# polimi-ispl/deep_prior_interpolation

Hardware: AMD Instinct MI355X
Metric: Adam iters/sec on 3D MultiRes-UNet (whole job over n_gpus; per_gpu beside it); recon SNR(dB) vs ref under config.snr_vs_reference (higher is better)
Workload: dtype f32

## Files before the change

deep_prior_interpolation_amd/csrc/conv_mfma.hip:

```cpp
#include "conv_kernels.h"

namespace {

typedef float f32x4 __attribute__((ext_vector_type(4)));

struct MArgs {
  const float* __restrict__ x;
  const float* __restrict__ chain;
  const float* __restrict__ w;
  const float* __restrict__ bias;
  float* __restrict__ y;
  double* __restrict__ partials;
  int Cin, Cout;
  int D, H, W;
  int ntd, nth, ntw;
  long w_out_stride, w_in_stride;
  int accumulate;
  int split_cps;
  const float* __restrict__ x2;
  const float* __restrict__ w2;
  int C2;
  long w2_co_stride, w2_c_stride;
  int xb, yb;
  int ny;
};

template <int KD, int NR, int NH, int S = 1>
struct Geo {
  static constexpr bool SLICES = (KD == 3 && NR >= 4);
  static constexpr int SD = KD == 3 ? S : 1;
  static constexpr int TZ = SLICES ? 4 : 1;
  static constexpr int TY = SLICES ? NR : 4 * NR;
  static constexpr int TW = 16 * NH;
  static constexpr int ID = (TZ - 1) * SD + KD;
  static constexpr int IH = (TY - 1) * S + 3;
  static constexpr int IW = (TW - 1) * S + 3;
  static constexpr int RS = (IW + 3) & ~3;
  static constexpr int DS0 = IH * RS;
  static constexpr int DS = (S == 1 && (RS % 32) == 4) ? DS0 + ((12 - (DS0 % 32)) + 32) % 32 : DS0;
  static constexpr int CS0 = ID * DS;
  static constexpr int CSM = S == 1 ? 16 : 1;
  static constexpr int CS = CS0 + ((CSM - (CS0 % 32)) + 32) % 32;
  static constexpr int TILE = ID * IH * IW;
  static constexpr int E = (TILE + 255) / 256;
  static constexpr int NROW = (NR - 1) * S + 3;
  static constexpr int NSTEP = KD * NROW;
  static constexpr int NB = 3 * NH;
};

__device__ __forceinline__ int xcd_tile(int bid, int ntiles) {
  const int q = ntiles >> 3, r = ntiles & 7, xcd = bid & 7, i = bid >> 3;
  return (xcd < r ? xcd * (q + 1) : r * (q + 1) + (xcd - r) * q) + i;
}

template <class G>
__device__ __forceinline__ void tile_slots(int tid, int id0, int ih0, int iw0, int D, int H, int W, int (&goff)[G::E], int (&loff)[G::E]) {
#pragma unroll
  for (int e = 0; e < G::E; ++e) {
    const int idx = tid + e * 256;
    const int col = idx % G::IW, row = idx / G::IW;
    const int hy = row % G::IH, dz = row / G::IH;
    const int gd = id0 + dz, gh = ih0 + hy, gw = iw0 + col;
    const bool ok = idx < G::TILE && gd >= 0 && gd < D && gh >= 0 && gh < H && gw >= 0 && gw < W;
    goff[e] = ok ? (gd * H + gh) * W + gw : -1;
    loff[e] = idx < G::TILE ? dz * G::DS + hy * G::RS + col : -1;
  }
}

template <class G>
__device__ __forceinline__ void stage_load(float (&sr)[4][G::E], const float* __restrict__ x, int Cin, size_t V, int c0,
                                           const int (&goff)[G::E], bool xb = false) {
  if (xb) {
#pragma unroll
    for (int c = 0; c < 4; ++c) {
      const int ci = min(c0 + c, Cin - 1);
      const __amdgpu_buffer_rsrc_t r = dpi_buffer_t(dpi_at(x, (size_t)ci * V, true), V, true);
#pragma unroll
      for (int e = 0; e < G::E; ++e) sr[c][e] = dpi_buffer_load_bf16_raw(r, goff[e]);
    }
    return;
  }
#pragma unroll
  for (int c = 0; c < 4; ++c) {
    const int ci = min(c0 + c, Cin - 1);
    const __amdgpu_buffer_rsrc_t r = dpi_buffer(x + (size_t)ci * V, V * sizeof(float));
#pragma unroll
    for (int e = 0; e < G::E; ++e) sr[c][e] = dpi_buffer_load(r, goff[e] * 4);
  }
}

template <class G>
__device__ __forceinline__ void stage_store(float* lds, const float (&sr_in)[4][G::E], const float* __restrict__ chain, int Cin, int c0,
                                            const int (&goff)[G::E], const int (&loff)[G::E], bool xb = false) {
  float sr[4][G::E];
#pragma unroll
  for (int c = 0; c < 4; ++c)
#pragma unroll
    for (int e = 0; e < G::E; ++e) sr[c][e] = sr_in[c][e];
  if (xb) {
#pragma unroll
    for (int c = 0; c < 4; ++c)
#pragma unroll
      for (int e = 0; e < G::E; ++e) sr[c][e] = dpi_widen_raw(sr[c][e]);
  }
  if (chain == nullptr) {
#pragma unroll
    for (int c = 0; c < 4; ++c)
// ... 11 lines not shown
      const float v = goff[e] >= 0 ? apply_chain(t, sr[c][e]) : sr[c][e];
      if ((e + 1) * 256 <= G::TILE || loff[e] >= 0) lds[c * G::CS + loff[e]] = v;
    }
  }
}

template <int KD, int NR, int NH>
struct GeoV2 {
  static constexpr int TY = 4 * NR, TW = 16 * NH;
  static constexpr int ID = KD == 3 ? 3 : 1, IH = (TY - 1) * 2 + 3;
  static constexpr int NQ = TW / 2 + 1;
  static constexpr int PW = 2 * NQ;
  static constexpr int RS = 2 * PW;
  static constexpr int DS = IH * RS;
  static constexpr int CS0 = ID * DS;
  static constexpr int CS = CS0 + ((16 - (CS0 % 32)) + 32) % 32;
  static constexpr int NV4 = ID * IH * NQ;
  static constexpr int E = (NV4 + 255) / 256;
};
template <class GV>
__device__ __forceinline__ void tile_slots_v(int tid, int id0, int ih0, int iw0, int D, int H, int W, int (&goff)[GV::E], int (&loff)[GV::E]) {
#pragma unroll
  for (int e = 0; e < GV::E; ++e) {
    const int idx = tid + e * 256;
    const int q = idx % GV::NQ, row = idx / GV::NQ;
    const int hy = row % GV::IH, dz = row / GV::IH;
    const int gd = id0 + dz, gh = ih0 + hy, gw = iw0 + 4 * q;
    const bool ok = idx < GV::NV4 && gd >= 0 && gd < D && gh >= 0 && gh < H && gw >= 0 && gw + 4 <= W;
    goff[e] = ok ? (gd * H + gh) * W + gw : -4;
    loff[e] = idx < GV::NV4 ? dz * GV::DS + hy * GV::RS + 2 * q : -1;
  }
}
template <class GV>
__device__ __forceinline__ void stage_load_v(f32x4 (&sv)[4][GV::E], const float* __restrict__ x, int Cin, size_t V, int c0, const int (&goff)[GV::E]) {
#pragma unroll
  for (int c = 0; c < 4; ++c) {
    const int ci = min(c0 + c, Cin - 1);
    const __amdgpu_buffer_rsrc_t r = dpi_buffer(x + (size_t)ci * V, V * sizeof(float));
#pragma unroll
    for (int e = 0; e < GV::E; ++e) sv[c][e] = __builtin_bit_cast(f32x4, __builtin_amdgcn_raw_buffer_load_b128(r, goff[e] * 4, 0, 0));
  }
}
template <class GV>
__device__ __forceinline__ void stage_store_v(float* lds, const f32x4 (&sv)[4][GV::E], const float* __restrict__ chain, int Cin, int c0,
                                              const int (&goff)[GV::E], const int (&loff)[GV::E]) {
  typedef float f32x2 __attribute__((ext_vector_type(2)));
  if (chain == nullptr) {
#pragma unroll
    for (int c = 0; c < 4; ++c)
#pragma unroll
      for (int e = 0; e < GV::E; ++e)
        if ((e + 1) * 256 <= GV::NV4 || loff[e] >= 0) {
          float* const p = lds + c * GV::CS + loff[e];
          *reinterpret_cast<f32x2*>(p) = (f32x2){sv[c][e][0], sv[c][e][2]};
          *reinterpret_cast<f32x2*>(p + GV::PW) = (f32x2){sv[c][e][1], sv[c][e][3]};
        }
    return;
  }
#pragma unroll
  for (int c = 0; c < 4; ++c) {
    const Chain t = load_chain(chain, min(c0 + c, Cin - 1));
#pragma unroll
    for (int e = 0; e < GV::E; ++e) {
      const float m = goff[e] >= 0 ? 1.f : 0.f;
      if ((e + 1) * 256 <= GV::NV4 || loff[e] >= 0) {
        float* const p = lds + c * GV::CS + loff[e];
        *reinterpret_cast<f32x2*>(p) = (f32x2){m * apply_chain(t, sv[c][e][0]), m * apply_chain(t, sv[c][e][2])};
        *reinterpret_cast<f32x2*>(p + GV::PW) = (f32x2){m * apply_chain(t, sv[c][e][1]), m * apply_chain(t, sv[c][e][3])};
      }
    }
  }
}

#ifdef DPI_TRACE
__device__ long long g_blk[8192][4];
__device__ long long g_trace[4][64];
#define TR(i) do { if (trc >= 0 && tid == 0) g_trace[trc][i] = clock64(); } while (0)
#define TRC(i) do { if (trc >= 0 && tid == 0 && (i) < 38) g_trace[trc][i] = clock64(); } while (0)
#else
#define TR(i)
#define TRC(i)
#endif
template <int KD, int NR, int NH, bool FLIP, int S = 1, int WPE = 2, bool PERSIST = false, bool TAILPACK = false, bool IOB = false, bool YLOOP = false,
          bool S2V = false>
__global__ __launch_bounds__(256, WPE) void conv_mfma_kernel(MArgs a) {
  static_assert(!YLOOP || (!PERSIST && !TAILPACK), "the channel-tile loop is built for the one-tile-per-workgroup variants without a packed tail");
  static_assert(!S2V || (S == 2 && !FLIP && !PERSIST && !TAILPACK && !IOB && NR < 4), "vectorised stride-2 staging: forward, fp32 tensors, row-split tiles");
  using GV = GeoV2<KD, NR < 4 ? NR : 2, NH>;
  if constexpr (!IOB) { a.xb = 0; a.yb = 0; }
  using G = Geo<KD, NR, NH, S>;
  constexpr int TAPS = KD * 9;
  constexpr int PD = (KD - 1) / 2;
  constexpr int NT = NR * NH;
  __shared__ __attribute__((aligned(16))) float lds[4 * (S2V ? GV::CS : G::CS)];
  __shared__ double red[4][16][2];

  const int tid = threadIdx.x, lane = tid & 63, wid = tid >> 6;
  const int lk = lane >> 4, lj = lane & 15;
  const int ntiles = a.ntd * a.nth * a.ntw;
  int vt0 = blockIdx.x, ytile = blockIdx.y;
  if constexpr (!PERSIST) {
    if (a.ny > 0) {
      const int q8 = ntiles >> 3, r8 = ntiles & 7, xcd = blockIdx.x & 7, j = blockIdx.x >> 3;
      const int i = YLOOP ? j : j / a.ny;
      ytile = YLOOP ? 0 : j - i * a.ny;
      if (i >= q8 + (xcd < r8 ? 1 : 0)) return;
      vt0 = i * 8 + xcd;
    }
  }
  int n0 = ytile * 16;
  const size_t V = (size_t)a.D * a.H * a.W;
  const int Do = (a.D + 2 * PD - KD) / G::SD + 1, Ho = (a.H - 1) / S + 1, Wo = (a.W - 1) / S + 1;
  const size_t Vo = (size_t)Do * Ho * Wo;
#ifdef DPI_TRACE
  const int trc = blockIdx.y != 0 ? -1 : blockIdx.x == 0 ? 0 : blockIdx.x == 1 ? 1 : blockIdx.x == 30 ? 2 : blockIdx.x == 50 ? 3 : -1;
  TR(0);
  if (tid == 0 && blockIdx.y == 0 && blockIdx.x < 8192) {
    g_blk[blockIdx.x][0] = wall_clock64();
    g_blk[blockIdx.x][2] = __builtin_amdgcn_s_getreg(63492);
    g_blk[blockIdx.x][3] = __builtin_amdgcn_s_getreg(63508);
  }
#endif
  auto tile_origin = [&](int vt, int& tile_id, int& od0, int& oh0, int& ow0) {
    tile_id = xcd_tile(vt, ntiles);
    int bt = tile_id;
    const int tw_i = bt % a.ntw; bt /= a.ntw;
    const int th_i = bt % a.nth; bt /= a.nth;
    od0 = bt * G::TZ; oh0 = th_i * G::TY; ow0 = tw_i * G::TW;
  };

  const int wz = G::SLICES ? wid : 0, wh = G::SLICES ? 0 : wid * NR;
  const int lbase = S2V ? lk * GV::CS + wh * 2 * GV::RS + lj : lk * G::CS + wz * G::SD * G::DS + wh * S * G::RS + lj * S;

  int co_w = n0 + lj;
  auto w_ptr = [&](int c0, bool& ok) {
    const int ci = c0 + lk;
    ok = co_w < a.Cout && ci < a.Cin;
    return a.w + (ok ? co_w : 0) * a.w_out_stride + (ok ? ci : 0) * a.w_in_stride;
  };
  auto load_w_raw = [&](float (&wn)[9], int c0, int kd) {
    bool ok;
    const float* __restrict__ wp = w_ptr(c0, ok);
#pragma unroll
    for (int t = 0; t < 9; ++t) wn[t] = wp[FLIP ? (TAPS - 1 - (kd * 9 + t)) : kd * 9 + t];
  };
  auto commit_w = [&](float (&wr)[TAPS], const float (&wn)[9], int c0, int kd) {
    const bool ok = co_w < a.Cout && c0 + lk < a.Cin;
#pragma unroll
    for (int t = 0; t < 9; ++t) wr[kd * 9 + t] = ok ? wn[t] : 0.f;
  };

  const int c_lo = a.split_cps ? (int)blockIdx.z * a.split_cps : 0;
  float* __restrict__ const ybase = a.y + (size_t)blockIdx.z * a.Cout * Vo;
  constexpr int EE = S2V ? GV::E : G::E;
  int goff[EE], loff[EE];
  float wr[TAPS], wn[9], sr[S2V ? 1 : 4][S2V ? 1 : G::E];
  f32x4 sv[S2V ? 4 : 1][S2V ? GV::E : 1];
  auto slots = [&](int od, int oh, int ow) {
    if constexpr (S2V) tile_slots_v<GV>(tid, od * G::SD - PD, oh * 2 - 1, ow * 2 - 4, a.D, a.H, a.W, goff, loff);
    else tile_slots<G>(tid, od * G::SD - PD, oh * S - 1, ow * S - 1, a.D, a.H, a.W, goff, loff);
  };
  auto sload = [&](int c0) {
    if constexpr (S2V) stage_load_v<GV>(sv, a.x, a.Cin, V, c0, goff);
    else stage_load<G>(sr, a.x, a.Cin, V, c0, goff, a.xb);
  };
  auto sstore = [&](int c0) {
    if constexpr (S2V) stage_store_v<GV>(lds, sv, a.chain, a.Cin, c0, goff, loff);
    else stage_store<G>(lds, sr, a.chain, a.Cin, c0, goff, loff, a.xb);
  };
  int vt = vt0, tile_id, od0, oh0, ow0;
  tile_origin(vt, tile_id, od0, oh0, ow0);
  slots(od0, oh0, ow0);
  sload(c_lo);
  {
    bool ok;
    const float* __restrict__ wp = w_ptr(c_lo, ok);
#pragma unroll
    for (int t = 0; t < TAPS; ++t) wr[t] = wp[FLIP ? (TAPS - 1 - t) : t];
#pragma unroll
    for (int t = 0; t < TAPS; ++t) wr[t] = ok ? wr[t] : 0.f;
  }

  constexpr int NTG = (TAPS + 3) / 4;
  const bool tail = TAILPACK && S == 1 && (a.Cin & 3) == 1 && (a.Cin > 4 || a.Cin == 1);
  const int cin_main = a.split_cps ? min(c_lo + a.split_cps, a.Cin) : (tail ? a.Cin - 1 : a.Cin);
  int ttoff[TAILPACK ? NTG : 1];
  float wt[TAILPACK ? NTG : 1];
  if constexpr (TAILPACK) {
#pragma unroll
    for (int g = 0; g < NTG; ++g) {
      const int t = 4 * g + lk;
      const int kd = t / 9, kh = (t / 3) % 3, kw = t % 3;
      ttoff[g] = t < TAPS ? kd * G::DS + kh * G::RS + kw : 0;
      wt[g] = 0.f;
    }
  }
  auto load_tail_w = [&]() {
    if constexpr (TAILPACK) {
      const bool ok = co_w < a.Cout;
      const float* __restrict__ wp = a.w + (ok ? co_w : 0) * a.w_out_stride + (a.Cin - 1) * a.w_in_stride;
#pragma unroll
      for (int g = 0; g < NTG; ++g) {
        const int t = 4 * g + lk < TAPS ? 4 * g + lk : TAPS - 1;
        wt[g] = wp[FLIP ? (TAPS - 1 - t) : t];
      }
    }
  };
  auto commit_tail_w = [&]() {
    if constexpr (TAILPACK) {
#pragma unroll
      for (int g = 0; g < NTG; ++g) wt[g] = (co_w < a.Cout && 4 * g + lk < TAPS) ? wt[g] : 0.f;
    }
  };

  for (;;) {
    const int vt_next = vt + (int)gridDim.x;
    const bool has_next = PERSIST && vt_next < ntiles;
    int tile_n = 0, od_n = 0, oh_n = 0, ow_n = 0;
    if (has_next) tile_origin(vt_next, tile_n, od_n, oh_n, ow_n);

    const int nyt = YLOOP ? a.ny : 1;
    for (int yt = 0; yt < nyt; ++yt) {
    if constexpr (YLOOP) {
      if (yt > 0) {
        n0 = yt * 16; co_w = n0 + lj;
        const bool ok = co_w < a.Cout && c_lo + lk < a.Cin;
#pragma unroll
        for (int t = 0; t < TAPS; ++t) wr[t] = ok ? wr[t] : 0.f;
      }
    }
    f32x4 acc[NT];
#pragma unroll
    for (int t = 0; t < NT; ++t) acc[t] = (f32x4){0.f, 0.f, 0.f, 0.f};
    if (a.accumulate) {
#pragma unroll
      for (int r = 0; r < 4; ++r) {
        const int co = n0 + 4 * lk + r;
#pragma unroll
        for (int t = 0; t < NT; ++t) {
          const int od = od0 + wz, oh = oh0 + wh + t / NH, ow = ow0 + (t % NH) * 16 + lj;
          if (co < a.Cout && od < Do && oh < Ho && ow < Wo) acc[t][r] = dpi_ld(ybase, (size_t)co * Vo + ((size_t)od * Ho + oh) * Wo + ow, a.yb);
        }
      }
    }

    TR(1);
    for (int c0 = c_lo; c0 < cin_main; c0 += 4) {
      if (!YLOOP || yt == 0) {
      __syncthreads();
      TRC(2 + (c0 / 4) * 4);
      sstore(c0);
      TRC(3 + (c0 / 4) * 4);
      __syncthreads();
      TRC(4 + (c0 / 4) * 4);
      }
      const bool more = c0 + 4 < cin_main;
      const bool tail_next = tail && !more;
      if (more || tail_next) sload(c0 + 4);
      else if (has_next) {
        slots(od_n, oh_n, ow_n);
        sload(c_lo);
      }
      float bc[G::NB], bn[G::NB];
      auto load_b = [&](float (&b)[G::NB], int step) {
        const int kd = step / G::NROW, ir = step % G::NROW;
#pragma unroll
        for (int h = 0; h < NH; ++h)
#pragma unroll
          for (int kw = 0; kw < 3; ++kw) {
            if constexpr (S2V)
              b[h * 3 + kw] = lds[lbase + kd * GV::DS + ir * GV::RS + h * 16 + (kw == 1 ? 2 : GV::PW + (kw == 0 ? 1 : 2))];
            else b[h * 3 + kw] = lds[lbase + kd * G::DS + ir * G::RS + h * 16 * S + kw];
          }
      };
      load_b(bc, 0);
      const int cn = more ? c0 + 4 : c_lo;
      if (tail_next) load_tail_w();
#pragma unroll
      for (int step = 0; step < G::NSTEP; ++step) {
        const int kd = step / G::NROW, ir = step % G::NROW;
        if (step + 1 < G::NSTEP) load_b(bn, step + 1);
        if constexpr (!YLOOP) { if (ir == 0) load_w_raw(wn, cn, kd); }
        if (WPE <= 2) __builtin_amdgcn_sched_barrier(0);
#pragma unroll
        for (int kw = 0; kw < 3; ++kw)
#pragma unroll
          for (int kh = 0; kh < 3; ++kh) {
            const int hr = (ir - kh) / S;
            if (ir - kh >= 0 && (ir - kh) % S == 0 && hr < NR) {
#pragma unroll
              for (int h = 0; h < NH; ++h)
                acc[hr * NH + h] = __builtin_amdgcn_mfma_f32_16x16x4f32(wr[(kd * 3 + kh) * 3 + kw], bc[h * 3 + kw], acc[hr * NH + h], 0, 0, 0);
            }
          }
        if (WPE <= 2) __builtin_amdgcn_sched_barrier(0);
#pragma unroll
        for (int i = 0; i < G::NB; ++i) bc[i] = bn[i];
        if constexpr (!YLOOP) { if (ir == G::NROW - 1) commit_w(wr, wn, cn, kd); }
      }
      if (tail_next) commit_tail_w();
      TRC(5 + (c0 / 4) * 4);
    }
    if constexpr (TAILPACK) {
      if (tail && cin_main == 0) { load_tail_w(); commit_tail_w(); }
      if (tail) {
        __syncthreads();
        sstore(cin_main);
        __syncthreads();
        if (has_next) {
          slots(od_n, oh_n, ow_n);
          sload(0);
        }
#pragma unroll
        for (int hr = 0; hr < NR; ++hr) {
          float tb[NH][NTG];
#pragma unroll
          for (int h = 0; h < NH; ++h)
#pragma unroll
            for (int g = 0; g < NTG; ++g) tb[h][g] = lds[lbase + ttoff[g] + hr * G::RS + h * 16];
#pragma unroll
          for (int g = 0; g < NTG; ++g)
#pragma unroll
            for (int h = 0; h < NH; ++h)
              acc[hr * NH + h] = __builtin_amdgcn_mfma_f32_16x16x4f32(wt[g], tb[h][g], acc[hr * NH + h], 0, 0, 0);
        }
      }
    }
    if constexpr (YLOOP) {
      if (yt + 1 < nyt) {
        const int con = (yt + 1) * 16 + lj, ci = c_lo + lk;
        const bool okn = con < a.Cout && ci < a.Cin;
        const float* __restrict__ wp = a.w + (okn ? con : 0) * a.w_out_stride + (okn ? ci : 0) * a.w_in_stride;
#pragma unroll
        for (int t = 0; t < TAPS; ++t) wr[t] = wp[FLIP ? (TAPS - 1 - t) : t];
      }
    }
    if constexpr (FLIP && !PERSIST) if (a.x2 != nullptr) {
      const __amdgpu_buffer_rsrc_t r2 = dpi_buffer_t(a.x2, (size_t)a.C2 * Vo, a.xb);
      int voff[NT];
#pragma unroll
      for (int t = 0; t < NT; ++t) {
        const int od = od0 + wz, oh = oh0 + wh + t / NH, ow = ow0 + (t % NH) * 16 + lj;
        voff[t] = (od < Do && oh < Ho && ow < Wo) ? (od * Ho + oh) * Wo + ow : -1;
      }
      const int nk2 = (a.C2 + 3) >> 2;
      auto load2 = [&](float (&b)[NT], float& wv, int kc) {
        const int c = kc * 4 + lk;
        const bool ok = c < a.C2 && co_w < a.Cout;
        const float wraw = a.w2[(ok ? co_w : 0) * a.w2_co_stride + (ok ? c : 0) * a.w2_c_stride];
        wv = ok ? wraw : 0.f;
        const int cbase = c * (int)Vo;
#pragma unroll
        for (int t = 0; t < NT; ++t)
          b[t] = a.xb ? dpi_buffer_load_bf16(r2, voff[t] >= 0 ? cbase + voff[t] : -1) : dpi_buffer_load(r2, voff[t] >= 0 ? (cbase + voff[t]) * 4 : -4);
      };
      float b0[NT], b1[NT], w0v, w1v;
      load2(b0, w0v, 0);
      for (int kc = 0; kc < nk2; kc += 2) {
        if (kc + 1 < nk2) load2(b1, w1v, kc + 1);
#pragma unroll
        for (int t = 0; t < NT; ++t) acc[t] = __builtin_amdgcn_mfma_f32_16x16x4f32(w0v, b0[t], acc[t], 0, 0, 0);
        if (kc + 1 < nk2) {
          if (kc + 2 < nk2) load2(b0, w0v, kc + 2);
#pragma unroll
          for (int t = 0; t < NT; ++t) acc[t] = __builtin_amdgcn_mfma_f32_16x16x4f32(w1v, b1[t], acc[t], 0, 0, 0);
        }
      }
    }
    TR(40);

    const bool interior = od0 + G::TZ <= Do && oh0 + G::TY <= Ho && ow0 + G::TW <= Wo && n0 + 16 <= a.Cout;
    const int vbase = ((od0 + wz) * Ho + oh0 + wh) * Wo + ow0 + lj;
#pragma unroll
    for (int r = 0; r < 4; ++r) {
      const int co = n0 + 4 * lk + r;
      const bool cok = co < a.Cout;
      const float bv = (a.bias && cok) ? a.bias[co] : 0.f;
      float* __restrict__ yc = dpi_at(ybase, (size_t)(cok ? co : 0) * Vo + vbase, a.yb);
      double s = 0.0, q = 0.0;
      if (a.yb) {
        const bool pairs = !(Wo & 1) && !(Vo & 1) && !((uintptr_t)ybase & 3);
#pragma unroll
        for (int t = 0; t < NT; ++t) {
          const int od = od0 + wz, oh = oh0 + wh + t / NH, ow = ow0 + (t % NH) * 16 + lj;
          const bool ok = interior || (cok && od < Do && oh < Ho && ow < Wo);
          const float v = dpi_round_bf16(acc[t][r] + bv);
          dpi_st_bf16_row(yc, (t / NH) * Wo + (t % NH) * 16, v, ok, pairs, lj);
          if (ok) { s += v; q += (double)v * v; }
        }
      } else if (interior) {
#pragma unroll
        for (int t = 0; t < NT; ++t) {
          const float v = acc[t][r] + bv;
          yc[(t / NH) * Wo + (t % NH) * 16] = v;
          if (a.partials) { s += v; q += (double)v * v; }
        }
      } else {
#pragma unroll
        for (int t = 0; t < NT; ++t) {
          const int od = od0 + wz, oh = oh0 + wh + t / NH, ow = ow0 + (t % NH) * 16 + lj;
          if (cok && od < Do && oh < Ho && ow < Wo) {
            const float v = acc[t][r] + bv;
            yc[(t / NH) * Wo + (t % NH) * 16] = v;
            s += v;
            q += (double)v * v;
          }
        }
      }
      if (a.partials) {
#pragma unroll
        for (int o = 8; o > 0; o >>= 1) { s += __shfl_xor(s, o, 64); q += __shfl_xor(q, o, 64); }
        if (lj == 0) { red[wid][4 * lk + r][0] = s; red[wid][4 * lk + r][1] = q; }
      }
    }
    if (a.partials) {
      __syncthreads();
      if (tid < 32) {
        const int c = tid >> 1, which = tid & 1;
        const double rsum = red[0][c][which] + red[1][c][which] + red[2][c][which] + red[3][c][which];
        if (n0 + c < a.Cout) a.partials[((size_t)tile_id * a.Cout + n0 + c) * 2 + which] = rsum;
      }
    }
    }
    TR(41);
    if (!has_next) break;
    vt = vt_next; tile_id = tile_n; od0 = od_n; oh0 = oh_n; ow0 = ow_n;
  }
#ifdef DPI_TRACE
  if (tid == 0 && blockIdx.y == 0 && blockIdx.x < 8192) g_blk[blockIdx.x][1] = wall_clock64();
#endif
}

struct BwMArgs {
  const float* __restrict__ x;
  const float* __restrict__ chain;
  const float* __restrict__ dy;
  float* __restrict__ ws;
  int Cin, Cout;
  int D, H, W;
  int ntd, nth, ntw, ntiles, tiles_per_chunk;
  int swap;
  int y0;
  int ngroups, nchunks;
  int xb, dyb;
};

template <int KD, int S, int NR, int NH, int NG = 1>
struct BwLds {
  using G = Geo<KD, NR, NH, S>;
  static constexpr int NTQ0 = (4 * KD * 9 + 15) / 16;
  static constexpr int LDSF = NG * (4 * G::CS > 4 * NTQ0 * 256 ? 4 * G::CS : 4 * NTQ0 * 256);
  static constexpr int DYRS = 4 * (4 * NH) + 4;
};

template <int KD, int S, int NR, int NH, int TC, int NG = 1, bool IOB = false>
__device__ __forceinline__ void conv_bwd_weight_mfma_body(const BwMArgs& a_in, float* __restrict__ lds, float* __restrict__ dyl_all, int first_group = -1) {
  BwMArgs a = a_in;
  if constexpr (!IOB) { a.xb = 0; a.dyb = 0; }
  static_assert(NG == 1 || TC == 0, "the column-trimmed tail is a single group");
#ifdef DPI_TRACE
  const int trc = (blockIdx.y == 0 && blockIdx.z == 0 && blockIdx.x < 4) ? (int)blockIdx.x : -1;
  int trn = 0;
#define TRW() do { if (trc >= 0 && threadIdx.x == 0 && trn < 64) g_trace[trc][trn++] = clock64(); } while (0)
#else
#define TRW()
#endif
  TRW();
  using G = Geo<KD, NR, NH, S>;
  constexpr int TAPS = KD * 9;
  constexpr int PD = (KD - 1) / 2;
  constexpr int NQ = (TC ? TC : 4) * TAPS;
  constexpr int NTQ = (NQ + 15) / 16;
  constexpr int KS = 4 * NH;
  constexpr int JP = KS / 4;
  constexpr int DYRS = BwLds<KD, S, NR, NH>::DYRS;

  const int tid = threadIdx.x, lane = tid & 63, wid = tid >> 6;
  const int lk = lane >> 4, lj = lane & 15;
  const int wch = lane >> 2, wp = lane & 3;
  float* __restrict__ dyw = dyl_all + wid * 16 * DYRS;
  int chunk = blockIdx.x, group = first_group >= 0 ? first_group : (int)blockIdx.y;
  if (first_group < 0 && a.ngroups > 0) {
    const int L = blockIdx.x, r = L >> 3;
    group = r % a.ngroups;
    chunk = (r / a.ngroups) * 8 + (L & 7);
    if (chunk >= a.nchunks) return;
  }
  const int c0 = (group + a.y0) * 4, n0 = blockIdx.z * 16;
  const size_t V = (size_t)a.D * a.H * a.W;
  const int Do = (a.D + 2 * PD - KD) / G::SD + 1, Ho = (a.H - 1) / S + 1, Wo = (a.W - 1) / S + 1;
  const size_t Vo = (size_t)Do * Ho * Wo;
  const int wz = G::SLICES ? wid : 0, wh = G::SLICES ? 0 : wid * NR;

  int toff[NTQ];
#pragma unroll
// ... 479 lines not shown
  for (int cls = 0; cls < NCLS; ++cls) {
    const int pw = cls & 1, ph = (cls >> 1) & 1, pd = KD == 3 ? (cls >> 2) & 1 : 0;
#pragma unroll
    for (int row = 0; row < 2; ++row) {
      const int id = KD == 3 ? 2 * md0 + pd : md0, ih = 2 * (mh0 + wid * 2 + row) + ph, iw = 2 * (mw0 + lj) + pw;
      if (id < a.D && ih < a.H && iw < a.W) {
#pragma unroll
        for (int r = 0; r < 4; ++r) {
          const int ci = n0 + 4 * lk + r;
          if (ci < a.Cin) {
            const size_t o = (size_t)ci * V + ((size_t)id * a.H + ih) * a.W + iw;
            dpi_st(a.dx, o, a.accumulate ? dpi_ld(a.dx, o, a.dxb) + acc[cls][row][r] : acc[cls][row][r], a.dxb);
          }
        }
      }
    }
  }
}

__global__ __launch_bounds__(256) void splitk_reduce_kernel(const float* __restrict__ ws, int nsplit, const float* __restrict__ bias,
                                                            float* __restrict__ y, int accumulate, double* __restrict__ partials,
                                                            int Cout, size_t Vo, size_t per, bool yb) {
  const int lane = threadIdx.x & 63, co = blockIdx.y * 4 + (threadIdx.x >> 6);
  if (co >= Cout) return;
  const size_t lo = (size_t)blockIdx.x * per, hi = lo + per < Vo ? lo + per : Vo;
  const float bv = bias ? bias[co] : 0.f;
  double sum = 0.0, sq = 0.0;
  for (size_t v = lo + lane; v < hi; v += 64) {
    float t = ws[(size_t)co * Vo + v];
    for (int sp = 1; sp < nsplit; ++sp) t += ws[((size_t)sp * Cout + co) * Vo + v];
    t += bv;
    if (accumulate) t += dpi_ld(y, (size_t)co * Vo + v, yb);
    t = dpi_stored(t, yb);
    dpi_st(y, (size_t)co * Vo + v, t, yb);
    sum += t; sq += (double)t * t;
  }
  if (partials) {
#pragma unroll
    for (int o = 32; o > 0; o >>= 1) { sum += __shfl_xor(sum, o, 64); sq += __shfl_xor(sq, o, 64); }
    if (lane == 0) { partials[((size_t)blockIdx.x * Cout + co) * 2] = sum; partials[((size_t)blockIdx.x * Cout + co) * 2 + 1] = sq; }
  }
}

}

static void dpi_mfma_variant(const dpi_conv_desc* d, int cout, int* nr, int* nh) {
  int Do, Ho, Wo;
  dpi_conv_out_dims(d, &Do, &Ho, &Wo);
  const int tz = d->kd == 3 ? 4 : 1, ty = d->kd == 3 ? 8 : 32;
  const long nb = (long)cdiv(Do, tz) * cdiv(Ho, ty) * cdiv(Wo, 32) * cdiv(cout, 16);
  if (nb >= 512 && d->stride == 1) { *nr = 8; *nh = 2; }
  else { *nr = 2; *nh = Wo > 16 ? 2 : 1; }
}

static bool dpi_mfma_half_tile(const dpi_conv_desc* d, bool flip) {
  const int cin = flip ? d->Cout : d->Cin, cout = flip ? d->Cin : d->Cout;
  int nr, nh;
  dpi_mfma_variant(d, cout, &nr, &nh);
  if (nr != 8 || d->kd != 3) return false;
  if (cin == 1) return true;
  if (cin <= 8) return false;
  return flip || ((cin & 3) == 1);
}

static int dpi_mfma_tiles(const dpi_conv_desc* d, int nr, int nh, int* ntd, int* nth, int* ntw) {
  int Do, Ho, Wo;
  dpi_conv_out_dims(d, &Do, &Ho, &Wo);
  const bool slices = d->kd == 3 && nr >= 4;
  const int tz = slices ? 4 : 1, ty = slices ? nr : 4 * nr;
  *ntd = cdiv(Do, tz); *nth = cdiv(Ho, ty); *ntw = cdiv(Wo, 16 * nh);
  return *ntd * *nth * *ntw;
}

struct MfmaTiling { int nr, nh, ntd, nth, ntw, ntiles; };
static MfmaTiling mfma_tiling(const dpi_conv_desc* d, bool flip) {
  MfmaTiling t{};
  dpi_mfma_variant(d, flip ? d->Cin : d->Cout, &t.nr, &t.nh);
  if (dpi_mfma_half_tile(d, flip)) t.nr = 4;
  t.ntiles = dpi_mfma_tiles(d, t.nr, t.nh, &t.ntd, &t.nth, &t.ntw);
  return t;
}
int dpi_conv_mfma_stat_blocks(const dpi_conv_desc* d, bool flip) { return mfma_tiling(d, flip).ntiles; }

template <int KD, bool FLIP, bool IOB = false>
static void launch_variant(const MArgs& a_in, int nr, int nh, int stride, dim3 grid_in, hipStream_t st) {
  if constexpr (!IOB) {
    if (a_in.xb || a_in.yb) { launch_variant<KD, FLIP, true>(a_in, nr, nh, stride, grid_in, st); return; }
  }
  const bool persistent = stride == 1 && nr == 8 && a_in.Cin > 8;
  MArgs a = a_in;
  dim3 grid = grid_in;
  if (!persistent && grid_in.y > 1) {
    a.ny = (int)grid_in.y;
    grid = dim3(8 * ((grid_in.x + 7) / 8) * grid_in.y, 1, grid_in.z);
  }
  if (stride == 2) {
    if constexpr (!FLIP) {
      if constexpr (!IOB) {
        static const bool s2v = getenv("DPI_NO_S2V") == nullptr;
        if (s2v && a.W % 4 == 0 && (((size_t)a.D * a.H * a.W) & 3) == 0 && ((uintptr_t)a.x & 15) == 0) {
          if (nh == 2) conv_mfma_kernel<KD, 2, 2, false, 2, 2, false, false, false, false, true><<<grid, 256, 0, st>>>(a);
          else conv_mfma_kernel<KD, 2, 1, false, 2, 2, false, false, false, false, true><<<grid, 256, 0, st>>>(a);
          return;
        }
      }
      if (nh == 2) conv_mfma_kernel<KD, 2, 2, false, 2, 2, false, false, IOB><<<grid, 256, 0, st>>>(a);
      else conv_mfma_kernel<KD, 2, 1, false, 2, 2, false, false, IOB><<<grid, 256, 0, st>>>(a);
    }
    return;
  }
  const bool tailpack = (a.Cin & 3) == 1 && (a.Cin > 4 || a.Cin == 1);
  if (nr == 4) {
    if constexpr (KD == 3) {
      if (tailpack) conv_mfma_kernel<KD, 4, 2, FLIP, 1, 3, false, true, IOB><<<grid, 256, 0, st>>>(a);
      else conv_mfma_kernel<KD, 4, 2, FLIP, 1, 3, false, false, IOB><<<grid, 256, 0, st>>>(a);
    }
    return;
  }
  if (nr == 8) {
    static const bool persist = getenv("DPI_NO_PERSIST") == nullptr;
    dim3 pg = grid;
    static const bool yloop = getenv("DPI_YLOOP") != nullptr && getenv("DPI_YLOOP")[0] == '1';
    if constexpr (KD == 3 && FLIP && !IOB) {
      if (yloop && a.Cin <= 4 && a.ny > 1 && a.split_cps == 0 && grid_in.z == 1) {
        conv_mfma_kernel<KD, 8, 2, FLIP, 1, 2, false, false, IOB, true><<<dim3(8 * ((grid_in.x + 7) / 8), 1, 1), 256, 0, st>>>(a);
        return;
      }
    }
    if (a.Cin <= 8) conv_mfma_kernel<KD, 8, 2, FLIP, 1, 3, false, false, IOB><<<grid, 256, 0, st>>>(a);
    else {
      if (persist && grid.x > 512) pg.x = 512;
      if (tailpack) conv_mfma_kernel<KD, 8, 2, FLIP, 1, 2, true, true, IOB><<<pg, 256, 0, st>>>(a);
      else conv_mfma_kernel<KD, 8, 2, FLIP, 1, 2, true, false, IOB><<<pg, 256, 0, st>>>(a);
    }
  }
  else if (nh == 2) conv_mfma_kernel<KD, 2, 2, FLIP, 1, 2, false, false, IOB><<<grid, 256, 0, st>>>(a);
  else conv_mfma_kernel<KD, 2, 1, FLIP, 1, 2, false, false, IOB><<<grid, 256, 0, st>>>(a);
}

#ifdef DPI_TRACE
extern "C" int dpi_debug_read_blocks(long long* out) { return (int)hipMemcpyFromSymbol(out, HIP_SYMBOL(g_blk), sizeof(long long) * 8192 * 4); }
extern "C" int dpi_debug_read_trace(long long* out) { return (int)hipMemcpyFromSymbol(out, HIP_SYMBOL(g_trace), sizeof(long long) * 4 * 64); }
#endif
static int g_splitk = getenv("DPI_SPLITK") ? atoi(getenv("DPI_SPLITK")) : 1;
extern "C" void dpi_set_splitk(int on) { g_splitk = on; }
static int dpi_mfma_splitk(const dpi_conv_desc* d, bool flip) {
  if (!g_splitk || d->k != 3) return 1;
  const int cin = flip ? d->Cout : d->Cin, cout = flip ? d->Cin : d->Cout;
  int nr, nh, a, b, c;
  dpi_mfma_variant(d, cout, &nr, &nh);
  if (nr != 2 || dpi_mfma_half_tile(d, flip)) return 1;
  const long wgs = (long)dpi_mfma_tiles(d, nr, nh, &a, &b, &c) * cdiv(cout, 16);
  const int chunks = cdiv(cin, 4);
  if (wgs > 512 || (wgs > 256 && chunks < 24)) return 1;
  long ns = 1536 / wgs;
  if (ns > chunks / 8) ns = chunks / 8;
  if (ns > 8) ns = 8;
  return ns < 2 ? 1 : (int)ns;
}
size_t dpi_conv_mfma_ws_floats(const dpi_conv_desc* d, bool flip) {
  const int ns = dpi_mfma_splitk(d, flip);
  if (ns < 2) return 0;
  int Do, Ho, Wo;
  dpi_conv_out_dims(d, &Do, &Ho, &Wo);
  return (size_t)ns * (flip ? d->Cin : d->Cout) * Do * Ho * Wo;
}

bool dpi_conv_mfma_second_ok(const dpi_conv_desc* d, bool flip, int C2, bool have_ws) {
  int Do, Ho, Wo;
  dpi_conv_out_dims(d, &Do, &Ho, &Wo);
  if (!flip || d->stride != 1 || C2 < 1 || ((size_t)C2 + 4) * Do * Ho * Wo * sizeof(float) >= ((size_t)1 << 31)) return false;
  int nr, nh;
  dpi_mfma_variant(d, d->Cin, &nr, &nh);
  if (nr == 8 && !dpi_mfma_half_tile(d, flip) && d->Cout > 8) return false;
  return !(have_ws && dpi_mfma_splitk(d, flip) > 1);
}

int dpi_conv_mfma_run(const dpi_conv_desc* d, const float* x, const float* chain, const float* w, const float* bias, float* y,
                      double* partials, bool flip, int accumulate, float* ws, size_t ws_floats, hipStream_t st, const MfmaSecond* sec) {
  const int taps = d->kd * 9;
  const int cin = flip ? d->Cout : d->Cin, cout = flip ? d->Cin : d->Cout;
  const long w_out = flip ? taps : (long)d->Cin * taps, w_in = flip ? (long)d->Cin * taps : taps;
  MArgs a{x, chain, w, bias, y, partials, cin, cout, d->D, d->H, d->W, 0, 0, 0, w_out, w_in, accumulate, 0, nullptr, nullptr, 0, 0, 0,
          dpi_io_in(d, flip), dpi_io_out(d, flip)};
  const MfmaTiling t = mfma_tiling(d, flip);
  const int nr = t.nr, nh = t.nh, ntiles = t.ntiles;
  a.ntd = t.ntd; a.nth = t.nth; a.ntw = t.ntw;
  dim3 grid(ntiles, cdiv(cout, 16));
  if (sec) { a.x2 = sec->x2; a.w2 = sec->w2; a.C2 = sec->C2; a.w2_co_stride = sec->w2_co_stride; a.w2_c_stride = sec->w2_c_stride; }
  const int nsplit = (ws && !sec) ? dpi_mfma_splitk(d, flip) : 1;
  if (nsplit > 1) {
    int Do, Ho, Wo;
    dpi_conv_out_dims(d, &Do, &Ho, &Wo);
    const size_t Vo = (size_t)Do * Ho * Wo;
    DPI_REQUIRE(ws_floats >= (size_t)nsplit * cout * Vo, "conv (split): workspace of %zu floats, need %zu", ws_floats, (size_t)nsplit * cout * Vo);
    a.split_cps = 4 * cdiv(cdiv(cin, 4), nsplit);
    a.y = ws; a.bias = nullptr; a.partials = nullptr; a.accumulate = 0; a.yb = 0;
    grid.z = cdiv(cin, a.split_cps);
    const int nz = (int)grid.z;
    if (d->kd == 3) { if (flip) launch_variant<3, true>(a, nr, nh, d->stride, grid, st); else launch_variant<3, false>(a, nr, nh, d->stride, grid, st); }
    else { if (flip) launch_variant<1, true>(a, nr, nh, d->stride, grid, st); else launch_variant<1, false>(a, nr, nh, d->stride, grid, st); }
    if (int e = dpi_check_launch("conv_mfma (split)")) return e;
    splitk_reduce_kernel<<<dim3(ntiles, cdiv(cout, 4)), 256, 0, st>>>(ws, nz, bias, y, accumulate, partials, cout, Vo, cdivz(Vo, (size_t)ntiles),
                                                                      dpi_io_out(d, flip));
    return dpi_check_launch("splitk_reduce");
  }
  if (d->kd == 3) { if (flip) launch_variant<3, true>(a, nr, nh, d->stride, grid, st); else launch_variant<3, false>(a, nr, nh, d->stride, grid, st); }
  else { if (flip) launch_variant<1, true>(a, nr, nh, d->stride, grid, st); else launch_variant<1, false>(a, nr, nh, d->stride, grid, st); }
  return dpi_check_launch("conv_mfma");
}

static bool mfma_bw_swap_better(const dpi_conv_desc* d) {
  if (d->stride != 1) return false;
  auto util = [](int rows, int staged) { return (double)rows / (16.0 * cdiv(rows, 16)) * staged / (4.0 * cdiv(staged, 4)); };
  return util(d->Cin, d->Cout) > 1.15 * util(d->Cout, d->Cin);
}

static int g_bw_want = getenv("DPI_BW_WANT") ? atoi(getenv("DPI_BW_WANT")) : 2304;
static int g_bw_xcd_order = getenv("DPI_BW_XCD_ORDER") ? atoi(getenv("DPI_BW_XCD_ORDER")) : 0;
extern "C" void dpi_set_bw_tuning(int want_workgroups, int xcd_order) {
  if (want_workgroups > 0) g_bw_want = want_workgroups;
  if (xcd_order >= 0) g_bw_xcd_order = xcd_order;
}
static size_t bw_extra_lds() { static const size_t v = getenv("DPI_BW_EXTRA_LDS") ? (size_t)atoi(getenv("DPI_BW_EXTRA_LDS")) * 1024 : 0; return v; }
struct MfmaBwPlan { int nchunks, tiles_per_chunk, ntiles, ntd, nth, ntw, nr, nh, npairs, nfull, ny; };
static int g_bw_pair = getenv("DPI_BW_PAIR") ? atoi(getenv("DPI_BW_PAIR")) : 2;
extern "C" void dpi_set_bw_pair(int mode) { if (mode >= 0 && mode <= 2) g_bw_pair = mode; }
static MfmaBwPlan mfma_bw_plan(const dpi_conv_desc* d, bool swap = false) {
  MfmaBwPlan p{};
  {
    const int staged = swap ? d->Cout : d->Cin, groups = cdiv(staged, 4);
    const bool s1k3 = d->stride == 1 && d->kd == 3;
    const int tailg = (s1k3 && (staged & 3) == 1) ? 1 : 0;
    p.nfull = groups - tailg;
    p.npairs = (g_bw_pair && s1k3 && !g_bw_xcd_order && p.nfull >= 2 && d->io == 0) ? p.nfull / 2 : 0;
    if (g_bw_pair == 2) {
      int a_, b_, c_;
      if (p.nfull < 4 || dpi_mfma_tiles(d, 8, 2, &a_, &b_, &c_) < 1024) p.npairs = 0;
    }
    p.ny = p.npairs ? p.npairs + (p.nfull & 1) + tailg : groups;
  }
  if (d->stride == 1) { p.nr = 8; p.nh = 2; }
  else { int Do, Ho, Wo; dpi_conv_out_dims(d, &Do, &Ho, &Wo); p.nr = 2; p.nh = Wo > 16 ? 2 : 1; }
  p.ntiles = dpi_mfma_tiles(d, p.nr, p.nh, &p.ntd, &p.nth, &p.ntw);
  const size_t per = (size_t)d->Cout * d->Cin * d->kd * 9;
  const size_t max_chunks_mem = per ? ((size_t)32 << 20) / per : 1;
  const size_t blocks_other = (size_t)p.ny * (swap ? cdiv(d->Cin, 16) : cdiv(d->Cout, 16));
  size_t want = (size_t)g_bw_want / blocks_other;
  if (want < 1) want = 1;
  if (want > (size_t)p.ntiles) want = p.ntiles;
  if (want > max_chunks_mem) want = max_chunks_mem;
  if (want < 1) want = 1;
  if (g_bw_xcd_order && want > 8) want = want / 8 * 8;
  p.tiles_per_chunk = (int)cdivz(p.ntiles, want);
  p.nchunks = cdiv(p.ntiles, p.tiles_per_chunk);
  return p;
}

size_t dpi_conv_bwd_weight_mfma_ws_floats(const dpi_conv_desc* d) {
  const int n0 = mfma_bw_plan(d, false).nchunks, n1 = mfma_bw_swap_better(d) ? mfma_bw_plan(d, true).nchunks : 0;
  return (size_t)(n0 > n1 ? n0 : n1) * d->Cout * d->Cin * d->kd * 9;
}
bool dpi_conv_bwd_weight_mfma_swapped(const dpi_conv_desc* d, bool chained) { return !chained && mfma_bw_swap_better(d); }

static int bf16_row_class(const void* base, int row_len, size_t channel_elems) {
  return ((row_len & 1) == 0 && (channel_elems & 1) == 0 && ((uintptr_t)base & 3) == 0) ? 1 : 2;
}

int dpi_conv_bwd_weight_mfma_run(const dpi_conv_desc* d, const float* x, const float* chain, const float* dy, float* dw, float* ws,
                                 hipStream_t st) {
  const bool swap = dpi_conv_bwd_weight_mfma_swapped(d, chain != nullptr);
  const MfmaBwPlan p = mfma_bw_plan(d, swap);
  BwMArgs a{x, chain, dy, ws, d->Cin, d->Cout, d->D, d->H, d->W, p.ntd, p.nth, p.ntw, p.ntiles, p.tiles_per_chunk, 0, 0, 0, p.nchunks,
            (d->io & DPI_IO_X_BF16) != 0, (d->io & DPI_IO_DY_BF16) != 0};
  dim3 grid(p.nchunks, cdiv(d->Cin, 4), cdiv(d->Cout, 16));
  if (swap) {
    a.x = dy; a.chain = nullptr; a.dy = x; a.Cin = d->Cout; a.Cout = d->Cin; a.swap = 1;
    a.xb = (d->io & DPI_IO_DY_BF16) != 0; a.dyb = (d->io & DPI_IO_X_BF16) != 0;
    grid = dim3(p.nchunks, cdiv(d->Cout, 4), cdiv(d->Cin, 16));
  }
// ... 105 lines not shown
```

Before: 34.28.

## Transpose MFMA operand order so each lane owns four contiguous outputs for vector stores

```diff
diff --git a/deep_prior_interpolation_amd/csrc/conv_mfma.hip b/deep_prior_interpolation_amd/csrc/conv_mfma.hip
--- a/deep_prior_interpolation_amd/csrc/conv_mfma.hip
+++ b/deep_prior_interpolation_amd/csrc/conv_mfma.hip
@@ -1,3 +1,4 @@
+#include <type_traits>
 #include "conv_kernels.h"
 
 namespace {
@@ -23,6 +24,7 @@
   long w2_co_stride, w2_c_stride;
   int xb, yb;
   int ny;
+  int vec;
 };
 
 template <int KD, int NR, int NH, int S = 1>
@@ -200,7 +202,7 @@
 #define TRC(i)
 #endif
 template <int KD, int NR, int NH, bool FLIP, int S = 1, int WPE = 2, bool PERSIST = false, bool TAILPACK = false, bool IOB = false, bool YLOOP = false,
-          bool S2V = false>
+          bool S2V = false, bool VEC = false>
 __global__ __launch_bounds__(256, WPE) void conv_mfma_kernel(MArgs a) {
   static_assert(!YLOOP || (!PERSIST && !TAILPACK), "the channel-tile loop is built for the one-tile-per-workgroup variants without a packed tail");
   static_assert(!S2V || (S == 2 && !FLIP && !PERSIST && !TAILPACK && !IOB && NR < 4), "vectorised stride-2 staging: forward, fp32 tensors, row-split tiles");
@@ -248,6 +250,8 @@
   };
 
   const int wz = G::SLICES ? wid : 0, wh = G::SLICES ? 0 : wid * NR;
+  const int wid_u = __builtin_amdgcn_readfirstlane(wid);
+  const int wz_u = G::SLICES ? wid_u : 0, wh_u = G::SLICES ? 0 : wid_u * NR;
   const int lbase = S2V ? lk * GV::CS + wh * 2 * GV::RS + lj : lk * G::CS + wz * G::SD * G::DS + wh * S * G::RS + lj * S;
 
   int co_w = n0 + lj;
@@ -347,17 +351,31 @@
         for (int t = 0; t < TAPS; ++t) wr[t] = ok ? wr[t] : 0.f;
       }
     }
+    auto row_ok = [&](int t) { return od0 + wz_u < Do && oh0 + wh_u + t / NH < Ho; };
+    auto group_nv = [&](int h, bool cok) { return cok ? min(max(Wo - (ow0 + 16 * h + 4 * lk), 0), 4) : 0; };
     f32x4 acc[NT];
 #pragma unroll
     for (int t = 0; t < NT; ++t) acc[t] = (f32x4){0.f, 0.f, 0.f, 0.f};
     if (a.accumulate) {
-#pragma unroll
-      for (int r = 0; r < 4; ++r) {
-        const int co = n0 + 4 * lk + r;
-#pragma unroll
-        for (int t = 0; t < NT; ++t) {
-          const int od = od0 + wz, oh = oh0 + wh + t / NH, ow = ow0 + (t % NH) * 16 + lj;
-          if (co < a.Cout && od < Do && oh < Ho && ow < Wo) acc[t][r] = dpi_ld(ybase, (size_t)co * Vo + ((size_t)od * Ho + oh) * Wo + ow, a.yb);
+      const int co = n0 + lj;
+      const bool cok = co < a.Cout;
+      int nv[NH];
+#pragma unroll
+      for (int h = 0; h < NH; ++h) nv[h] = group_nv(h, cok);
+      const float* __restrict__ yin = dpi_at(ybase, (size_t)(cok ? co : 0) * Vo + ((od0 + wz) * Ho + oh0 + wh) * Wo + ow0 + 4 * lk, a.yb);
+#pragma unroll
+      for (int t = 0; t < NT; ++t) {
+        if (!row_ok(t)) continue;
+        const int i = (t / NH) * Wo + (t % NH) * 16;
+        if constexpr (VEC) {
+          if (nv[t % NH] > 0) {
+            const float4 v = dpi_ld4(yin, i, a.yb, false);
+            acc[t] = (f32x4){v.x, v.y, v.z, v.w};
+          }
+        } else {
+#pragma unroll
+          for (int e = 0; e < 4; ++e)
+            if (e < nv[t % NH]) acc[t][e] = dpi_ld(yin, i + e, a.yb);
         }
       }
     }
@@ -408,7 +426,7 @@
             if (ir - kh >= 0 && (ir - kh) % S == 0 && hr < NR) {
 #pragma unroll
               for (int h = 0; h < NH; ++h)
-                acc[hr * NH + h] = __builtin_amdgcn_mfma_f32_16x16x4f32(wr[(kd * 3 + kh) * 3 + kw], bc[h * 3 + kw], acc[hr * NH + h], 0, 0, 0);
+                acc[hr * NH + h] = __builtin_amdgcn_mfma_f32_16x16x4f32(bc[h * 3 + kw], wr[(kd * 3 + kh) * 3 + kw], acc[hr * NH + h], 0, 0, 0);
             }
           }
         if (WPE <= 2) __builtin_amdgcn_sched_barrier(0);
@@ -440,7 +458,7 @@
           for (int g = 0; g < NTG; ++g)
 #pragma unroll
             for (int h = 0; h < NH; ++h)
-              acc[hr * NH + h] = __builtin_amdgcn_mfma_f32_16x16x4f32(wt[g], tb[h][g], acc[hr * NH + h], 0, 0, 0);
+              acc[hr * NH + h] = __builtin_amdgcn_mfma_f32_16x16x4f32(tb[h][g], wt[g], acc[hr * NH + h], 0, 0, 0);
         }
       }
     }
@@ -477,58 +495,72 @@
       for (int kc = 0; kc < nk2; kc += 2) {
         if (kc + 1 < nk2) load2(b1, w1v, kc + 1);
 #pragma unroll
-        for (int t = 0; t < NT; ++t) acc[t] = __builtin_amdgcn_mfma_f32_16x16x4f32(w0v, b0[t], acc[t], 0, 0, 0);
+        for (int t = 0; t < NT; ++t) acc[t] = __builtin_amdgcn_mfma_f32_16x16x4f32(b0[t], w0v, acc[t], 0, 0, 0);
         if (kc + 1 < nk2) {
           if (kc + 2 < nk2) load2(b0, w0v, kc + 2);
 #pragma unroll
-          for (int t = 0; t < NT; ++t) acc[t] = __builtin_amdgcn_mfma_f32_16x16x4f32(w1v, b1[t], acc[t], 0, 0, 0);
+          for (int t = 0; t < NT; ++t) acc[t] = __builtin_amdgcn_mfma_f32_16x16x4f32(b1[t], w1v, acc[t], 0, 0, 0);
         }
       }
     }
     TR(40);
 
     const bool interior = od0 + G::TZ <= Do && oh0 + G::TY <= Ho && ow0 + G::TW <= Wo && n0 + 16 <= a.Cout;
-    const int vbase = ((od0 + wz) * Ho + oh0 + wh) * Wo + ow0 + lj;
-#pragma unroll
-    for (int r = 0; r < 4; ++r) {
-      const int co = n0 + 4 * lk + r;
+    {
+      const int co = n0 + lj;
       const bool cok = co < a.Cout;
       const float bv = (a.bias && cok) ? a.bias[co] : 0.f;
+      const int vbase = ((od0 + wz) * Ho + oh0 + wh) * Wo + ow0 + 4 * lk;
       float* __restrict__ yc = dpi_at(ybase, (size_t)(cok ? co : 0) * Vo + vbase, a.yb);
-      double s = 0.0, q = 0.0;
-      if (a.yb) {
-        const bool pairs = !(Wo & 1) && !(Vo & 1) && !((uintptr_t)ybase & 3);
+      const bool pairs = !(Wo & 1) && !(Vo & 1) && !((uintptr_t)ybase & 3);
+      double s[4] = {0.0, 0.0, 0.0, 0.0}, q[4] = {0.0, 0.0, 0.0, 0.0};
+      auto tiles_out = [&](auto inner) {
+        constexpr bool INNER = decltype(inner)::value;
+        int nv[NH];
+#pragma unroll
+        for (int h = 0; h < NH; ++h) nv[h] = INNER ? 4 : group_nv(h, cok);
 #pragma unroll
         for (int t = 0; t < NT; ++t) {
-          const int od = od0 + wz, oh = oh0 + wh + t / NH, ow = ow0 + (t % NH) * 16 + lj;
-          const bool ok = interior || (cok && od < Do && oh < Ho && ow < Wo);
-          const float v = dpi_round_bf16(acc[t][r] + bv);
-          dpi_st_bf16_row(yc, (t / NH) * Wo + (t % NH) * 16, v, ok, pairs, lj);
-          if (ok) { s += v; q += (double)v * v; }
-        }
-      } else if (interior) {
-#pragma unroll
-        for (int t = 0; t < NT; ++t) {
-          const float v = acc[t][r] + bv;
-          yc[(t / NH) * Wo + (t % NH) * 16] = v;
-          if (a.partials) { s += v; q += (double)v * v; }
-        }
-      } else {
-#pragma unroll
-        for (int t = 0; t < NT; ++t) {
-          const int od = od0 + wz, oh = oh0 + wh + t / NH, ow = ow0 + (t % NH) * 16 + lj;
-          if (cok && od < Do && oh < Ho && ow < Wo) {
-            const float v = acc[t][r] + bv;
-            yc[(t / NH) * Wo + (t % NH) * 16] = v;
-            s += v;
-            q += (double)v * v;
+          if (!INNER && !row_ok(t)) continue;
+          const int i = (t / NH) * Wo + (t % NH) * 16, n = nv[t % NH];
+          float v[4];
+#pragma unroll
+          for (int e = 0; e < 4; ++e) v[e] = dpi_stored(acc[t][e] + bv, a.yb);
+          if constexpr (VEC) {
+            if (INNER || n > 0) dpi_st4(yc, i, make_float4(v[0], v[1], v[2], v[3]), a.yb, false);
+          } else if (a.yb) {
+#pragma unroll
+            for (int e = 0; e < 4; e += 2) {
+              unsigned short* const p = reinterpret_cast<unsigned short*>(yc) + i + e;
+              if (pairs) { if (INNER || e < n) *reinterpret_cast<unsigned*>(p) = dpi_pack_bf16(v[e], v[e + 1]); }
+              else {
+                if (INNER || e < n) p[0] = dpi_f32_to_bf16(v[e]);
+                if (INNER || e + 1 < n) p[1] = dpi_f32_to_bf16(v[e + 1]);
+              }
+            }
+          } else {
+#pragma unroll
+            for (int e = 0; e < 4; ++e)
+              if (INNER || e < n) yc[i + e] = v[e];
+          }
+          if (a.partials) {
+#pragma unroll
+            for (int e = 0; e < 4; ++e) {
+              const float u = (INNER || e < n) ? v[e] : 0.f;
+              s[e] += u; q[e] += (double)u * u;
+            }
           }
         }
-      }
+      };
+      if (interior) tiles_out(std::true_type{}); else tiles_out(std::false_type{});
       if (a.partials) {
 #pragma unroll
-        for (int o = 8; o > 0; o >>= 1) { s += __shfl_xor(s, o, 64); q += __shfl_xor(q, o, 64); }
-        if (lj == 0) { red[wid][4 * lk + r][0] = s; red[wid][4 * lk + r][1] = q; }
+        for (int e = 0; e < 4; ++e) {
+          s[e] += __shfl_xor(s[e], 32, 64); q[e] += __shfl_xor(q[e], 32, 64);
+          s[e] += __shfl_xor(s[e], 16, 64); q[e] += __shfl_xor(q[e], 16, 64);
+        }
+        const double s2 = (s[0] + s[2]) + (s[1] + s[3]), q2 = (q[0] + q[2]) + (q[1] + q[3]);
+        if (lk == 0) { red[wid][lj][0] = s2; red[wid][lj][1] = q2; }
       }
     }
     if (a.partials) {
@@ -1174,10 +1206,13 @@
 }
 int dpi_conv_mfma_stat_blocks(const dpi_conv_desc* d, bool flip) { return mfma_tiling(d, flip).ntiles; }
 
-template <int KD, bool FLIP, bool IOB = false>
+template <int KD, bool FLIP, bool IOB = false, bool VEC = false>
 static void launch_variant(const MArgs& a_in, int nr, int nh, int stride, dim3 grid_in, hipStream_t st) {
   if constexpr (!IOB) {
-    if (a_in.xb || a_in.yb) { launch_variant<KD, FLIP, true>(a_in, nr, nh, stride, grid_in, st); return; }
+    if (a_in.xb || a_in.yb) { launch_variant<KD, FLIP, true, VEC>(a_in, nr, nh, stride, grid_in, st); return; }
+  }
+  if constexpr (!VEC) {
+    if (a_in.vec) { launch_variant<KD, FLIP, IOB, true>(a_in, nr, nh, stride, grid_in, st); return; }
   }
   const bool persistent = stride == 1 && nr == 8 && a_in.Cin > 8;
   MArgs a = a_in;
@@ -1191,21 +1226,21 @@
       if constexpr (!IOB) {
         static const bool s2v = getenv("DPI_NO_S2V") == nullptr;
         if (s2v && a.W % 4 == 0 && (((size_t)a.D * a.H * a.W) & 3) == 0 && ((uintptr_t)a.x & 15) == 0) {
-          if (nh == 2) conv_mfma_kernel<KD, 2, 2, false, 2, 2, false, false, false, false, true><<<grid, 256, 0, st>>>(a);
-          else conv_mfma_kernel<KD, 2, 1, false, 2, 2, false, false, false, false, true><<<grid, 256, 0, st>>>(a);
+          if (nh == 2) conv_mfma_kernel<KD, 2, 2, false, 2, 2, false, false, false, false, true, VEC><<<grid, 256, 0, st>>>(a);
+          else conv_mfma_kernel<KD, 2, 1, false, 2, 2, false, false, false, false, true, VEC><<<grid, 256, 0, st>>>(a);
           return;
         }
       }
-      if (nh == 2) conv_mfma_kernel<KD, 2, 2, false, 2, 2, false, false, IOB><<<grid, 256, 0, st>>>(a);
-      else conv_mfma_kernel<KD, 2, 1, false, 2, 2, false, false, IOB><<<grid, 256, 0, st>>>(a);
+      if (nh == 2) conv_mfma_kernel<KD, 2, 2, false, 2, 2, false, false, IOB, false, false, VEC><<<grid, 256, 0, st>>>(a);
+      else conv_mfma_kernel<KD, 2, 1, false, 2, 2, false, false, IOB, false, false, VEC><<<grid, 256, 0, st>>>(a);
     }
     return;
   }
   const bool tailpack = (a.Cin & 3) == 1 && (a.Cin > 4 || a.Cin == 1);
   if (nr == 4) {
     if constexpr (KD == 3) {
-      if (tailpack) conv_mfma_kernel<KD, 4, 2, FLIP, 1, 3, false, true, IOB><<<grid, 256, 0, st>>>(a);
-      else conv_mfma_kernel<KD, 4, 2, FLIP, 1, 3, false, false, IOB><<<grid, 256, 0, st>>>(a);
+      if (tailpack) conv_mfma_kernel<KD, 4, 2, FLIP, 1, 3, false, true, IOB, false, false, VEC><<<grid, 256, 0, st>>>(a);
+      else conv_mfma_kernel<KD, 4, 2, FLIP, 1, (FLIP && !IOB) ? 4 : 3, false, false, IOB, false, false, VEC><<<grid, 256, 0, st>>>(a);
     }
     return;
   }
@@ -1215,19 +1250,19 @@
     static const bool yloop = getenv("DPI_YLOOP") != nullptr && getenv("DPI_YLOOP")[0] == '1';
     if constexpr (KD == 3 && FLIP && !IOB) {
       if (yloop && a.Cin <= 4 && a.ny > 1 && a.split_cps == 0 && grid_in.z == 1) {
-        conv_mfma_kernel<KD, 8, 2, FLIP, 1, 2, false, false, IOB, true><<<dim3(8 * ((grid_in.x + 7) / 8), 1, 1), 256, 0, st>>>(a);
+        conv_mfma_kernel<KD, 8, 2, FLIP, 1, 2, false, false, IOB, true, false, VEC><<<dim3(8 * ((grid_in.x + 7) / 8), 1, 1), 256, 0, st>>>(a);
         return;
       }
     }
-    if (a.Cin <= 8) conv_mfma_kernel<KD, 8, 2, FLIP, 1, 3, false, false, IOB><<<grid, 256, 0, st>>>(a);
+    if (a.Cin <= 8) conv_mfma_kernel<KD, 8, 2, FLIP, 1, 3, false, false, IOB, false, false, VEC><<<grid, 256, 0, st>>>(a);
     else {
       if (persist && grid.x > 512) pg.x = 512;
-      if (tailpack) conv_mfma_kernel<KD, 8, 2, FLIP, 1, 2, true, true, IOB><<<pg, 256, 0, st>>>(a);
-      else conv_mfma_kernel<KD, 8, 2, FLIP, 1, 2, true, false, IOB><<<pg, 256, 0, st>>>(a);
-    }
-  }
-  else if (nh == 2) conv_mfma_kernel<KD, 2, 2, FLIP, 1, 2, false, false, IOB><<<grid, 256, 0, st>>>(a);
-  else conv_mfma_kernel<KD, 2, 1, FLIP, 1, 2, false, false, IOB><<<grid, 256, 0, st>>>(a);
+      if (tailpack) conv_mfma_kernel<KD, 8, 2, FLIP, 1, 2, true, true, IOB, false, false, VEC><<<pg, 256, 0, st>>>(a);
+      else conv_mfma_kernel<KD, 8, 2, FLIP, 1, 2, true, false, IOB, false, false, VEC><<<pg, 256, 0, st>>>(a);
+    }
+  }
+  else if (nh == 2) conv_mfma_kernel<KD, 2, 2, FLIP, 1, 2, false, false, IOB, false, false, VEC><<<grid, 256, 0, st>>>(a);
+  else conv_mfma_kernel<KD, 2, 1, FLIP, 1, 2, false, false, IOB, false, false, VEC><<<grid, 256, 0, st>>>(a);
 }
 
 #ifdef DPI_TRACE
@@ -1268,6 +1303,13 @@
   return !(have_ws && dpi_mfma_splitk(d, flip) > 1);
 }
 
+static int mfma_vec_ok(const dpi_conv_desc* d, const void* y, bool yb) {
+  static const bool on = getenv("DPI_NO_VEC_EPILOGUE") == nullptr;
+  int Do, Ho, Wo;
+  dpi_conv_out_dims(d, &Do, &Ho, &Wo);
+  return on && Wo % 4 == 0 && ((uintptr_t)y & (yb ? 7u : 15u)) == 0;
+}
+
 int dpi_conv_mfma_run(const dpi_conv_desc* d, const float* x, const float* chain, const float* w, const float* bias, float* y,
                       double* partials, bool flip, int accumulate, float* ws, size_t ws_floats, hipStream_t st, const MfmaSecond* sec) {
   const int taps = d->kd * 9;
@@ -1279,6 +1321,7 @@
   const int nr = t.nr, nh = t.nh, ntiles = t.ntiles;
   a.ntd = t.ntd; a.nth = t.nth; a.ntw = t.ntw;
   dim3 grid(ntiles, cdiv(cout, 16));
+  a.vec = mfma_vec_ok(d, y, a.yb != 0);
   if (sec) { a.x2 = sec->x2; a.w2 = sec->w2; a.C2 = sec->C2; a.w2_co_stride = sec->w2_co_stride; a.w2_c_stride = sec->w2_c_stride; }
   const int nsplit = (ws && !sec) ? dpi_mfma_splitk(d, flip) : 1;
   if (nsplit > 1) {
@@ -1288,6 +1331,7 @@
     DPI_REQUIRE(ws_floats >= (size_t)nsplit * cout * Vo, "conv (split): workspace of %zu floats, need %zu", ws_floats, (size_t)nsplit * cout * Vo);
     a.split_cps = 4 * cdiv(cdiv(cin, 4), nsplit);
     a.y = ws; a.bias = nullptr; a.partials = nullptr; a.accumulate = 0; a.yb = 0;
+    a.vec = mfma_vec_ok(d, ws, false);
     grid.z = cdiv(cin, a.split_cps);
     const int nz = (int)grid.z;
     if (d->kd == 3) { if (flip) launch_variant<3, true>(a, nr, nh, d->stride, grid, st); else launch_variant<3, false>(a, nr, nh, d->stride, grid, st); }
```

After: 34.51, median of 2. No clear change (+0.7%).
